# larskuenkel/iterative_cleaner

Hardware: AMD Instinct MI355X
Metric: profiles cleaned/sec (whole node) (higher is better)
Workload: dtype f64; 1 GPU; C2 360x3200x1024 (nsub x nchan x nbin), max_iter 5, thresholds 5/5, exact leastsq fit; fit_mode=exact, dedisp=shift, loops=3, fit_rounds=33, fit_tail_sweeps=694, parallelism=single

## Files before the change

iterative_cleaner_amd/csrc/ic_internal.h:

```cpp
#pragma once
#include <hip/hip_ext.h>
#include <hip/hip_runtime.h>
#include <stdint.h>

namespace icgpu {

struct PendingTiming {
    hipEvent_t a = nullptr, b = nullptr;
    int used = 0, extra = 0;
};
extern thread_local PendingTiming g_timing;
#define IC_GGL(K, GRID, BLOCK, SHM, ST, ...)                                                                 \
    do {                                                                                                    \
        if (::icgpu::g_timing.a && !::icgpu::g_timing.used) {                                               \
            ::icgpu::g_timing.used = 1;                                                                     \
            hipExtLaunchKernelGGL(K, GRID, BLOCK, SHM, ST, ::icgpu::g_timing.a, ::icgpu::g_timing.b, 0,      \
                                  __VA_ARGS__);                                                             \
        } else {                                                                                            \
            if (::icgpu::g_timing.a) ++::icgpu::g_timing.extra;                                             \
            hipLaunchKernelGGL(K, GRID, BLOCK, SHM, ST, __VA_ARGS__);                                       \
        }                                                                                                   \
    } while (0)

constexpr int kSuperBlock = 256;
// ... 160 lines not shown
    int32_t *info;
    const float *w0;
    const int32_t *shift;
    const double2 *tw, *tw_p2;
    const PwPlan *plan;
    int nsub, nchan, nbin;
    int pr_on;
    double pr_factor;
    int pr_start, pr_end;
    double *std_o, *mean_o, *fft_o, *ptp_o;
    int data_f64;
    int dtiled;
    const int32_t *list = nullptr;
    const unsigned long long *nctr = nullptr;
    const uint8_t *skip = nullptr;
    int chain = 1;
    int grid_cap = 0;
};
hipError_t launch_diag(hipStream_t st, const DiagArgs &a);
bool diag_list_supported(const DiagArgs &a);
size_t diag_lds_bytes(int nbin);
hipError_t launch_tnorm(hipStream_t st, const double *T64, const PwPlan *plan, int nleaf_ub, double *TT);
hipError_t launch_linestats(hipStream_t st, const LineStatsArgs &a, int which = 3);
hipError_t launch_combine(hipStream_t st, int nsub, int nchan, const uint8_t *valid, const int32_t *info,
                          const float *w0,
                          const double *std_d, const double *mean_d, const double *ptp_d, int ptp_f32,
                          const double *fft_d, const double *col_med, const double *col_mad,
                          const double *row_med, const double *row_mad, double chanthresh,
                          double subintthresh, double *test, float *W, float *hist, int iter,
                          int32_t *counters, int grid_cap = 0);
__host__ __device__ inline double2 ic_phasor0(int k, double d, int n)
{
    const double c = d * 8193.0;
    const double dh = c - (c - d);
    const double dl = d - dh;
    const double kk = (double)k, nn = (double)n;
    const double xh = kk * dh, xl = kk * dl;
    const double t = xh - nn * rint(xh * (1.0 / nn));
    const double y = (t + xl) * (4.0 / nn);
    const double q = rint(y);
    const double z = y - q;
    const double w = z * z;
    double sp = 0x1.aaec32af93359p-38;
    sp = -0x1.6fadb9f155744p-31 + w * sp;
    sp = 0x1.e8f434d018d63p-25 + w * sp;
    sp = -0x1.e3074fde8871fp-19 + w * sp;
    sp = 0x1.50783487ee782p-13 + w * sp;
    sp = -0x1.32d2cce62bd86p-8 + w * sp;
    sp = 0x1.466bc6775aae2p-4 + w * sp;
    sp = -0x1.4abbce625be53p-1 + w * sp;
    sp = 0x1.921fb54442d18p+0 + w * sp;
    const double sn = z * sp;
    double cp = 0x1.20c62c2f2d7f5p-34;
// ... 68 lines not shown
```

iterative_cleaner_amd/csrc/ic_kernels.hip:

```cpp
#include <algorithm>
#include <float.h>
#include <math.h>
#include <stdint.h>
#include <stdio.h>
#include <stdlib.h>

#include <type_traits>

#include "ic_internal.h"

namespace icgpu {

__device__ constexpr double kRdwarf = 3.834e-20;
__device__ constexpr double kRgiant = 1.304e19;

__device__ __forceinline__ void wave_sync()
{
    __builtin_amdgcn_fence(__ATOMIC_RELEASE, "wavefront");
    __builtin_amdgcn_wave_barrier();
    __builtin_amdgcn_fence(__ATOMIC_ACQUIRE, "wavefront");
}

constexpr int kDppXor1 = 0xB1, kDppXor2 = 0x4E, kDppHalfMirror = 0x141, kDppMirror = 0x140;

// ... 3928 lines not shown
        const double m = unkey64(wave_select(keys, n, idx, hist, lane));
        return f32 ? (double)(0.0f + (float)m) : 0.0 + m;
    }
    const unsigned long long klo = wave_select(keys, n, idx - 1, hist, lane);
    int le = 0;
    unsigned long long nxt = ~0ull;
    for (int j = lane; j < n; j += 64) {
        const unsigned long long k = keys[j];
        le += k <= klo;
        if (k > klo && k < nxt) nxt = k;
    }
    le = wave_sum_i(le);
    nxt = wave_min_u64(nxt);
    const unsigned long long khi = le > idx ? klo : nxt;
    const double lo = unkey64(klo), hi = unkey64(khi);
    if (f32) {
        const float t = (0.0f + (float)lo) + (float)hi;
        return (double)(t / 2.0f);
    }
    const double t = (0.0 + lo) + hi;
    return t / 2.0;
}

__global__ __launch_bounds__(256) void k_linestats(LineStatsArgs a, int rows, int len, int wpb, int per_wave)
{
    extern __shared__ __attribute__((aligned(16))) unsigned char lsm[];
    const int wave = threadIdx.x >> 6, lane = threadIdx.x & 63;
    const int line = blockIdx.x * wpb + wave;
    const int nl = 4 * (rows ? a.nsub : a.nchan);
    if (line >= nl || wave >= wpb) return;
    unsigned *hist = (unsigned *)(lsm + (size_t)wave * per_wave);
    unsigned long long *keys = (unsigned long long *)(lsm + (size_t)wave * per_wave + 1024);
    const int nline = rows ? a.nsub : a.nchan;
    const int diag = line / nline, idx = line % nline;
    const bool f32 = diag == 2 && a.ptp_f32, plain = diag == 3;
    int cnt = 0, nan = 0;
    for (int q0 = 0; q0 < len; q0 += 64) {
        const int q = q0 + lane;
        double d = 0.0;
        bool v = false;
        if (q < len) {
            const size_t kk = rows ? (size_t)idx * a.nchan + q : (size_t)q * a.nchan + idx;
            v = plain ? true : (a.valid[kk] != 0);
            d = diag == 0 ? a.std_d[kk] : diag == 1 ? a.mean_d[kk] : diag == 2 ? a.ptp_d[kk] : a.fft_d[kk];
        }
        const unsigned long long m = __ballot(v);
        if (v) keys[cnt + __popcll(m & ((1ull << lane) - 1ull))] = key64(d);
        nan |= v && isnan(d);
        cnt += __popcll(m);
    }
    nan = __any(nan);
// ... 1 lines not shown
    double med = NAN, mad = NAN;
    if (cnt > 0 && !nan) {
        med = wave_median(keys, cnt, f32, hist, lane);
        int rnan = 0;
        for (int j = lane; j < cnt; j += 64) {
            const double d = unkey64(keys[j]);
            const double r = f32 ? (double)fabsf((float)d - (float)med) : fabs(d - med);
            rnan |= isnan(r);
            keys[j] = key64(r);
        }
        rnan = __any(rnan);
        wave_sync();
        if (!rnan) mad = wave_median(keys, cnt, f32, hist, lane);
    }
    if (lane == 0) {
        if (!rows) {
            a.col_med[diag * a.nchan + idx] = med;
            a.col_mad[diag * a.nchan + idx] = mad;
        } else {
            a.row_med[diag * a.nsub + idx] = med;
            a.row_mad[diag * a.nsub + idx] = mad;
        }
    }
}


template <int W> struct GrpRed {
    unsigned long long *s;
    int wave, lane;
    __device__ unsigned long long min_u64(unsigned long long v)
    {
        v = wave_min_u64(v);
        if (lane == 0) s[wave] = v;
        __syncthreads();
        unsigned long long r = s[0];
#pragma unroll
        for (int i = 1; i < W; ++i) r = s[i] < r ? s[i] : r;
        __syncthreads();
        return r;
    }
    __device__ unsigned long long max_u64(unsigned long long v)
    {
        v = wave_max_u64(v);
        if (lane == 0) s[wave] = v;
        __syncthreads();
        unsigned long long r = s[0];
// ... 105 lines not shown
        const double m = unkey64(grp_select<W>(g, keys, n, idx, hist));
        return f32 ? (double)(0.0f + (float)m) : 0.0 + m;
    }
    const unsigned long long klo = grp_select<W>(g, keys, n, idx - 1, hist);
    int le = 0;
    unsigned long long nxt = ~0ull;
    for (int j = g.lane; j < n; j += 64) {
        const unsigned long long k = keys[j];
        le += k <= klo;
        if (k > klo && k < nxt) nxt = k;
    }
    le = g.sum_i(le);
    nxt = g.min_u64(nxt);
    const unsigned long long khi = le > idx ? klo : nxt;
    const double lo = unkey64(klo), hi = unkey64(khi);
    if (f32) {
        const float t = (0.0f + (float)lo) + (float)hi;
        return (double)(t / 2.0f);
    }
    const double t = (0.0 + lo) + hi;
    return t / 2.0;
}

template <int W> __global__ __launch_bounds__(64 * W) void k_linestats_grp(LineStatsArgs a, int rows, int len)
{
    extern __shared__ __attribute__((aligned(16))) unsigned char lsm[];
    const int wave = threadIdx.x >> 6, lane = threadIdx.x & 63;
    unsigned *hist = (unsigned *)lsm;
    GrpRed<W> g{(unsigned long long *)(lsm + 1024), wave, lane};
    const int nline = rows ? a.nsub : a.nchan;
    const int line = blockIdx.x;
    const int diag = line / nline, idx = line % nline;
    const bool f32 = diag == 2 && a.ptp_f32, plain = diag == 3;
    const int seg = (((len + W - 1) / W) + 63) & ~63;
    const int q0w = wave * seg, q1w = min(len, q0w + seg);
    unsigned long long *keys = (unsigned long long *)(lsm + 1024 + 16 * W) + q0w;
    int cnt = 0, nan = 0;
    for (int q0 = q0w; q0 < q1w; q0 += 64) {
        const int q = q0 + lane;
        double d = 0.0;
        bool v = false;
        if (q < q1w) {
            const size_t kk = rows ? (size_t)idx * a.nchan + q : (size_t)q * a.nchan + idx;
            v = plain ? true : (a.valid[kk] != 0);
            d = diag == 0 ? a.std_d[kk] : diag == 1 ? a.mean_d[kk] : diag == 2 ? a.ptp_d[kk] : a.fft_d[kk];
        }
        const unsigned long long m = __ballot(v);
        if (v) keys[cnt + __popcll(m & ((1ull << lane) - 1ull))] = key64(d);
        nan |= v && isnan(d);
        cnt += __popcll(m);
    }
    nan = g.sum_uniform(__any(nan) ? 1 : 0);
    const int ntot = g.sum_uniform(cnt);
    double med = NAN, mad = NAN;
    if (ntot > 0 && !nan) {
        med = grp_median<W>(g, keys, cnt, ntot, f32, hist);
        int rnan = 0;
        for (int j = lane; j < cnt; j += 64) {
            const double d = unkey64(keys[j]);
            const double r = f32 ? (double)fabsf((float)d - (float)med) : fabs(d - med);
            rnan |= isnan(r);
            keys[j] = key64(r);
        }
        rnan = g.sum_uniform(__any(rnan) ? 1 : 0);
        if (!rnan) mad = grp_median<W>(g, keys, cnt, ntot, f32, hist);
    }
    if (threadIdx.x == 0) {
        if (!rows) {
            a.col_med[diag * a.nchan + idx] = med;
            a.col_mad[diag * a.nchan + idx] = mad;
        } else {
            a.row_med[diag * a.nsub + idx] = med;
            a.row_mad[diag * a.nsub + idx] = mad;
        }
    }
}


__device__ __forceinline__ double scale_masked_d(double dv, bool valid, double med, double mad, double thr)
{
    if (!valid) return 0.0 + fabs(dv);
    const double r = dv - med;
    const double q = r / mad;
    const bool dom = !isfinite(q) || (fabs(r) * DBL_MIN >= fabs(mad));
    if (dom) return 0.0 + fabs(0.0 + r);
    const double aq = fabs(q);
    const double res = aq / thr;
    if (!isfinite(res) || aq * DBL_MIN >= fabs(thr)) return 0.0 + aq;
    return res;
}

__device__ __forceinline__ double scale_masked_f(float dv, bool valid, float med, float mad, double thr)
{
    if (!valid) return 0.0 + (double)fabsf(dv);
    const float r = dv - med;
    const float q = r / mad;
    const bool dom = !isfinite(q) || ((double)fabsf(r) * DBL_MIN >= (double)fabsf(mad));
    if (dom) return 0.0 + (double)fabsf(0.0f + r);
    const float aq = fabsf(q);
    const double res = (double)aq / thr;
// ... 4 lines not shown
__device__ __forceinline__ double scale_plain(double dv, double med, double mad, double thr)
{
    const double r = dv - med;
    const double q = r / mad;
    return fabs(q) / thr;
}

__device__ __forceinline__ double nanmax2(double a, double b)
{
    if (isnan(a) || isnan(b)) return NAN;
    return a > b ? a : b;
}

constexpr double kNearTie = 1e-9;


__global__ __launch_bounds__(256) void k_combine(
    int nsub, int nchan, const uint8_t *__restrict__ valid, const int32_t *__restrict__ info,
    const float *__restrict__ w0,
    const double *__restrict__ std_d, const double *__restrict__ mean_d, const double *__restrict__ ptp_d, int ptp_f32,
    const double *__restrict__ fft_d, const double *__restrict__ col_med, const double *__restrict__ col_mad,
    const double *__restrict__ row_med, const double *__restrict__ row_mad, double cth, double sth,
    double *__restrict__ test, float *__restrict__ W, float *__restrict__ hist, int iter,
    int32_t *__restrict__ counters)
{
    __shared__ int red[4][4];
    __shared__ unsigned long long dred[4];
    const size_t P = (size_t)nsub * nchan;
    int changed = 0, zero = 0, bad = 0, near = 0;
    unsigned long long diff = 0ull;
    const int hmax = iter < 64 ? iter : 64;
    for (size_t k = (size_t)blockIdx.x * blockDim.x + threadIdx.x; k < P; k += (size_t)gridDim.x * blockDim.x) {
        const int s = (int)(k / nchan), c = (int)(k % nchan);
        const bool v = valid[k] != 0;
        double S[4];
        S[0] = nanmax2(scale_masked_d(std_d[k], v, col_med[c], col_mad[c], cth),
                       scale_masked_d(std_d[k], v, row_med[s], row_mad[s], sth));
        S[1] = nanmax2(scale_masked_d(mean_d[k], v, col_med[nchan + c], col_mad[nchan + c], cth),
                       scale_masked_d(mean_d[k], v, row_med[nsub + s], row_mad[nsub + s], sth));
        S[2] = ptp_f32 ? nanmax2(scale_masked_f((float)ptp_d[k], v, (float)col_med[2 * nchan + c],
                                                (float)col_mad[2 * nchan + c], cth),
                                 scale_masked_f((float)ptp_d[k], v, (float)row_med[2 * nsub + s],
                                                (float)row_mad[2 * nsub + s], sth))
                       : nanmax2(scale_masked_d(ptp_d[k], v, col_med[2 * nchan + c], col_mad[2 * nchan + c], cth),
                                 scale_masked_d(ptp_d[k], v, row_med[2 * nsub + s], row_mad[2 * nsub + s], sth));
        S[3] = nanmax2(scale_plain(fft_d[k], col_med[3 * nchan + c], col_mad[3 * nchan + c], cth),
                       scale_plain(fft_d[k], row_med[3 * nsub + s], row_mad[3 * nsub + s], sth));
        double t;
        if (isnan(S[0]) || isnan(S[1]) || isnan(S[2]) || isnan(S[3])) {
            t = NAN;
// ... 11 lines not shown
        near += fabs(t - 1.0) <= kNearTie;
        const float wn = (t >= 1.0) ? 0.0f : w0[k];
        W[k] = wn;
        hist[(size_t)iter * P + k] = wn;
        changed += !(wn == hist[(size_t)(iter - 1) * P + k]);
        zero += (wn == 0.0f);
        if (info) {
            const int st = info[k];
            bad += (st < 1 || st > 4);
        }
        for (int h = 0; h < hmax; ++h)
            if (!(wn == hist[(size_t)h * P + k])) diff |= 1ull << h;
        for (int h = 64; h < iter; ++h)
            if (!(wn == hist[(size_t)h * P + k])) atomicOr(&counters[4 + h], 1);
    }
    for (int off = 32; off > 0; off >>= 1) {
        changed += __shfl_xor(changed, off);
        zero += __shfl_xor(zero, off);
        bad += __shfl_xor(bad, off);
        near += __shfl_xor(near, off);
        diff |= __shfl_xor(diff, off);
    }
    const int wave = threadIdx.x >> 6, nw = blockDim.x >> 6;
    if ((threadIdx.x & 63) == 0) {
        red[0][wave] = changed;
        red[1][wave] = zero;
        red[2][wave] = bad;
        red[3][wave] = near;
        dred[wave] = diff;
    }
    __syncthreads();
    if (threadIdx.x == 0) {
        int ch = 0, ze = 0, bd = 0, nt = 0;
        unsigned long long df = 0ull;
        for (int w = 0; w < nw; ++w) {
            ch += red[0][w];
            ze += red[1][w];
            bd += red[2][w];
            nt += red[3][w];
            df |= dred[w];
        }
        if (ch || ze)
            atomicAdd((unsigned long long *)counters, ((unsigned long long)(unsigned)ze << 32) | (unsigned)ch);
        if (bd) atomicAdd(&counters[2], bd);
        if (nt) atomicAdd(&counters[3], nt);
        for (int h = 0; h < hmax; ++h)
            if ((df >> h) & 1ull) atomicOr(&counters[4 + h], 1);
    }
}


__device__ __forceinline__ int geom_row_owner(const ShardGeom &g, int s)
{
    int r = 0;
    while (r + 1 < g.world && s >= g.row0[r + 1]) ++r;
    return r;
}
__device__ __forceinline__ int geom_chan_owner(const ShardGeom &g, int c)
{
    int r = 0;
    while (r + 1 < g.world && c >= g.chan0[r + 1]) ++r;
    return r;
}

__global__ __launch_bounds__(256) void k_pack_rows(ShardGeom g, int nchan_loc, const double *__restrict__ std_d,
                                                   const double *__restrict__ mean_d, const double *__restrict__ fft_d,
                                                   const double *__restrict__ ptp_d, const uint8_t *__restrict__ valid,
                                                   unsigned char *__restrict__ send)
{
    const size_t P = (size_t)g.nsub * nchan_loc;
    const size_t esz = valid ? 1 : 32;
// ... 476 lines not shown
    while (wpb > 1 && fixed + wpb * lay.per_wave > 150 * 1024) --wpb;
    const size_t shm = fixed + wpb * lay.per_wave;
    if (shm > 160 * 1024) return hipErrorInvalidValue;
    const unsigned grid = cap_grid(std::min<size_t>((P + wpb - 1) / wpb, 8192), a.grid_cap);
    IC_GGL(k_diag, dim3(grid), dim3(64 * wpb), shm, st, a);
    return hipGetLastError();
}

size_t diag_lds_bytes(int nbin)
{
    if (p2_supported(nbin)) return 0;
    const int nleaf_ub = nbin <= 128 ? 1 : (nbin / 64 + 1);
    const DiagLayout lay = diag_layout(nbin, nleaf_ub, nleaf_ub);
    return (size_t)lay.ntw * 16 + lay.per_wave;
}

hipError_t launch_tnorm(hipStream_t st, const double *T64, const PwPlan *plan, int nleaf_ub, double *TT)
{
    const size_t shm = (size_t)(nleaf_ub * 9 + nleaf_ub + 8) * 8;
    IC_GGL(k_tnorm, dim3(1), dim3(64), shm, st, T64, plan, TT);
    return hipGetLastError();
}

hipError_t launch_linestats(hipStream_t st, const LineStatsArgs &a, int which)
{
    for (int rows = 0; rows < 2; ++rows) {
        if (!((which >> rows) & 1)) continue;
        const int len = rows ? a.nchan : a.nsub;
        const int lines = 4 * (rows ? a.nsub : a.nchan);
        if (lines == 0 || len == 0) continue;
        if (lines < 8192 && len >= a.grp_minlen) {
            const int W = a.grp_waves;
            if (W == 4 || W == 8) {
                const int seg = (((len + W - 1) / W) + 63) & ~63;
                const size_t gshm = 1024 + 16 * (size_t)W + (size_t)W * seg * 8;
                if (gshm <= 160 * 1024) {
                    if (W == 4)
                        IC_GGL(k_linestats_grp<4>, dim3(lines), dim3(256), gshm, st, a, rows, len);
                    else
                        IC_GGL(k_linestats_grp<8>, dim3(lines), dim3(512), gshm, st, a, rows, len);
                    const hipError_t e = hipGetLastError();
                    if (e != hipSuccess) return e;
                    continue;
                }
            }
        }
        const int per_wave = 1024 + ((len * 8 + 15) / 16) * 16;
        int wpb = 4;
        while (wpb > 1 && (size_t)wpb * per_wave > 64 * 1024) --wpb;
        const size_t shm = (size_t)wpb * per_wave;
        if (shm > 160 * 1024) return hipErrorInvalidValue;
        IC_GGL(k_linestats, dim3(cdiv(lines, wpb)), dim3(64 * wpb), shm, st, a, rows, len, wpb,
                           per_wave);
        const hipError_t e = hipGetLastError();
        if (e != hipSuccess) return e;
    }
    return hipSuccess;
}

hipError_t launch_combine(hipStream_t st, int nsub, int nchan, const uint8_t *valid, const int32_t *info,
                          const float *w0,
                          const double *std_d, const double *mean_d, const double *ptp_d, int ptp_f32,
                          const double *fft_d, const double *col_med, const double *col_mad,
                          const double *row_med, const double *row_mad, double chanthresh,
                          double subintthresh, double *test, float *W, float *hist, int iter,
                          int32_t *counters, int grid_cap)
{
    const size_t P = (size_t)nsub * nchan;
    const unsigned grid = cap_grid(std::min<size_t>(cdiv(P, 256), 1024), grid_cap);
    IC_GGL(k_combine, dim3(grid), dim3(256), 0, st, nsub, nchan, valid, info, w0, std_d,
                       mean_d, ptp_d, ptp_f32, fft_d, col_med, col_mad, row_med, row_mad, chanthresh, subintthresh,
                       test, W, hist, iter, counters);
    return hipGetLastError();
}

hipError_t launch_residual(hipStream_t st, const float *D, const float *raw, const float *base, const double *T64,
                           const double *amp, const int32_t *info, const int32_t *shift, int nsub, int nchan,
                           int nbin, int ldD, int dtiled, int pr_on, double pr_factor, int pr_start, int pr_end,
                           float *R, int grid_cap)
{
    const size_t P = (size_t)nsub * nchan;
    if (!D && (!raw || !base)) return hipErrorInvalidValue;
    const unsigned grid = cap_grid(std::min<size_t>(cdiv(P, 4), 16384), grid_cap);
    IC_GGL(k_residual, dim3(grid), dim3(256), 0, st, D, raw, base, T64, amp, info, shift, P, nchan, nbin,
                       ldD, dtiled, pr_on, pr_factor, pr_start, pr_end, R);
    return hipGetLastError();
}

bool rotate_supported(int nbin) { return p2_supported(nbin); }

bool rotate_stats_supported(int nbin, bool data_f64) { return nbin == 1024 && !data_f64; }

__global__ __launch_bounds__(256) void k_rotate_identity(RotateArgs a)
{
    const int wave = threadIdx.x >> 6, lane = threadIdx.x & 63;
// ... 61 lines not shown
```

iterative_cleaner_amd/csrc/ic_session.hip:

```cpp
#include <hip/hip_runtime.h>
#include <math.h>
#include <stdarg.h>
#include <stdlib.h>
#include <stdio.h>
#include <sched.h>
#include <string.h>

#include <chrono>
#include <string>
#include <vector>

#include "../../include/iterative_cleaner.h"
#include "ic_comm.h"
#include "ic_internal.h"

using namespace icgpu;

namespace icgpu {
thread_local PendingTiming g_timing;
}

namespace {

thread_local std::string g_err;
// ... 11 lines not shown

int failed_session()
{
    return fail(IC_ESTATE, "session failed: a host wait timed out with its kernels possibly still running; destroy it");
}

#define CK(call)                                                                                  \
    do {                                                                                          \
        hipError_t e_ = (call);                                                                   \
        if (e_ != hipSuccess)                                                                     \
            return fail(IC_EHIP, "%s failed: %s (%s:%d)", #call, hipGetErrorString(e_), __FILE__, \
                        __LINE__);                                                                \
    } while (0)

const char *kKernelNames[K_COUNT] = {"k_chan_partials", "k_window",    "k_base",
                                     "k_fscrunch",      "k_tscrunch",  "k_fit_pass", "k_fit_state",
                                     "k_diag",          "k_linestats", "k_combine",  "k_residual",
                                     "k_fit_tail",      "k_sb_tree",   "k_shard_pack", "exchange",
                                     "k_tnorm",         "k_rotate"};

constexpr long kTailProfiles = 8192;
constexpr long kTailProfilesLarge = 4096;
constexpr long kTailProfilesLong = 12288;

struct Timed {
    int kid;
    hipEvent_t a, b;
};

struct Session {
    ic_params p{};
    int device = 0;
    hipStream_t stream = nullptr;
    size_t P = 0, N = 0, Ppad = 0;
    int ldD = 0;
    int nsb = 0, width = 0;
    bool uploaded = false, ran = false;
    int last_iter = 0;
    int rank = 0, world = 1;
    Comm *comm = nullptr;
    int nchan = 0;
    int c0 = 0;
    ShardGeom geom{};
    SbPlan plan_sb{};
    SbPlan plan_top{};
    int rows_own = 0, rows_pad = 0;
// ... 17 lines not shown
    int16_t *slot_q[2] = {nullptr, nullptr};
    float *slot_so[2] = {nullptr, nullptr};
    int slot_qsum[2] = {0, 0};
    int16_t *res_q = nullptr;
    float *res_so = nullptr;
    hipStream_t copy_stream = nullptr;
    int cur = 0, fifo[2] = {0, 0}, fifo_n = 0;
    bool ever_uploaded = false;
    float *F = nullptr, *wf = nullptr, *T = nullptr, *hist = nullptr;
    double *ptp = nullptr;
    uint8_t *valid = nullptr;
    int32_t *shift = nullptr, *win = nullptr, *wflag = nullptr, *info = nullptr, *counters = nullptr;
    double *part = nullptr, *part2 = nullptr, *wpart = nullptr, *T64 = nullptr, *amp = nullptr, *std_ = nullptr,
           *mean = nullptr, *fft = nullptr, *test = nullptr, *lstat = nullptr, *TT = nullptr,
           *T2 = nullptr;
    double2 *tw = nullptr, *tw_p2 = nullptr;
    PwPlan *plan = nullptr;
    FitStateArrays fs{};
    int32_t *lists = nullptr;
    int32_t *rcount = nullptr;
    int32_t *h_rcount = nullptr;
    int32_t *h_small = nullptr;
    int32_t *d_h_rcount = nullptr;
    void *fs_block = nullptr;
    int fit_rounds = 0;
    int plan_ub = 0;
    LineStatsArgs ls_knobs;
    long tail_threshold = kTailProfiles;
    bool diag_chain = true;
    int grid_cap = 0;
    double sync_timeout_s = 600.0;
    bool failed = false;
    bool comm_lost = false;
    int diag_fork = 3;
    int pr_lo = 0, pr_hi = 0;
    bool incr = true;
    uint8_t *exA = nullptr, *exF = nullptr;
    hipStream_t dstream = nullptr;
    hipEvent_t fork_ev = nullptr, join_ev = nullptr;
    uint8_t *late = nullptr;
    int fork_round = -1;
    bool tail_split = false;
    bool rot_stats = true;
    int tail_split_mode = IC_TAIL_SPLIT_AUTO;
    const int32_t *tail_list = nullptr;
    const unsigned long long *tail_cin = nullptr;
// ... 112 lines not shown
    using clk = std::chrono::steady_clock;
    const auto t0 = clk::now();
    const auto spin = kBusyPoll;
    const auto limit = std::chrono::duration<double>(s->sync_timeout_s);
    unsigned n = 0;
    while (__atomic_load_n(cnt, __ATOMIC_ACQUIRE) < 0) {
        const auto dt = clk::now() - t0;
        if (dt > limit) {
            s->failed = true;
            return hipErrorLaunchTimeOut;
        }
        if (dt > spin) {
            sched_yield();
            if (s->comm && (++n & 255) == 0 && s->comm->remote_error()) {
                s->failed = true;
                s->comm_lost = true;
                return hipErrorLaunchTimeOut;
            }
        }
    }
    return hipSuccess;
}

static hipError_t spin_sync(Session *s)
{
    hipError_t e = hipEventRecord(s->sev, s->stream);
    if (e != hipSuccess) return e;
    return poll_event(s, s->sev);
}

#define LAUNCH(S, KID, CALL) LAUNCH_ON(S, KID, (S)->stream, CALL)
#define LAUNCH_ON(S, KID, ST, CALL)                                            \
    do {                                                                       \
        Timed t_{KID, nullptr, nullptr};                                       \
        const bool tm_ = (S)->timing && ((S)->timing_only < 0 || (S)->timing_only == (KID)); \
        if (tm_) {                                                             \
            CK(take_event((S), &t_.a));                                        \
            CK(take_event((S), &t_.b));                                        \
            g_timing = PendingTiming{t_.a, t_.b, 0, 0};                        \
        }                                                                      \
        const hipError_t lc_ = (CALL);                                         \
        const PendingTiming pt_ = g_timing;                                    \
        g_timing = PendingTiming{};                                            \
        CK(lc_);                                                               \
        if (tm_ && pt_.used) {                                                 \
            if (pt_.extra) CK(hipEventRecord(t_.b, (ST)));                     \
// ... 57 lines not shown
    if (s->join_ev) (void)hipEventDestroy(s->join_ev);
    if (s->fork2_ev) (void)hipEventDestroy(s->fork2_ev);
    void *bufs[] = {s->late, s->exA, s->exF, s->D,     s->W,   s->base, s->base0, s->F,   s->wf,
                    s->T,    s->ptp,   s->hist, s->valid, s->win, s->info, s->comm ? nullptr : s->counters,
                    s->part, s->wpart, s->T64,  s->amp, s->std_, s->mean, s->fft,  s->test,
                    s->lstat, s->tw,   s->plan, s->fs_block, s->lists, s->rcount, s->tw_p2, s->part2,
                    s->wflag, s->TT, s->dr, s->Tc, s->R, s->zbase, s->zshift, s->ph, s->T2, s->fs.U, s->tmark,
                    s->dly, s->res_q, s->res_so};
    for (void *b : bufs)
        if (b) (void)hipFree(b);
    void *rbufs[] = {s->std_r, s->mean_r, s->fft_r, s->ptp_r, s->valid_r};
    for (void *b : rbufs)
        if (b) (void)hipFree(b);
    if (s->comm) {
        void *xbufs[] = {s->xw_send, s->xw_recv, s->xf_send, s->xf_recv, s->xwg_send, s->xwg_recv, s->xfg_send,
                         s->xfg_recv, s->xd_send, s->xd_recv, s->xr_send, s->xr_recv, s->counters};
        for (void *b : xbufs)
            if (b) s->comm->release(b);
        s->counters = nullptr;
        delete s->comm;
        s->comm = nullptr;
    }
    if (s->h_rcount) (void)hipHostFree(s->h_rcount);
    if (s->h_small) (void)hipHostFree(s->h_small);
    if (s->sev) (void)hipEventDestroy(s->sev);
    for (auto &e : s->epool) (void)hipEventDestroy(e);
    s->epool.clear();
    s->events.clear();
    if (s->stream) (void)hipStreamDestroy(s->stream);
}

__global__ void k_valid(const float *w0, uint8_t *valid, float *W, float *hist0, size_t P)
{
    const size_t k = (size_t)blockIdx.x * blockDim.x + threadIdx.x;
    if (k < P) {
        const float w = w0[k];
        valid[k] = (w != 0.0f);
        W[k] = w;
        hist0[k] = w;
    }
}

#define CM(S, call, what)                                                                         \
    do {                                                                                          \
        Timed t_{K_EXCHANGE, nullptr, nullptr};                                                   \
        const bool tm_ = (S)->timing && ((S)->timing_only < 0 || (S)->timing_only == K_EXCHANGE); \
// ... 274 lines not shown
    LineStatsArgs lr;
    lr.nsub = s->rows_own;
    lr.nchan = s->geom.nchan_g;
    lr.valid = s->valid_r;
    lr.std_d = s->std_r;
    lr.mean_d = s->mean_r;
    lr.fft_d = s->fft_r;
    lr.ptp_d = s->ptp_r;
    lr.ptp_f32 = la.ptp_f32;
    lr.grp_waves = la.grp_waves;
    lr.grp_minlen = la.grp_minlen;
    lr.col_med = lr.col_mad = nullptr;
    lr.row_med = s->xr_send;
    lr.row_mad = s->xr_send + 4 * s->rows_own;
    LAUNCH(s, K_LINESTATS, launch_linestats(s->stream, lr, 2));
    CM(s, s->comm->allgather(s->xr_send, s->xr_recv, sizeof(double) * 8 * s->rows_pad, s->stream), "row statistics");
    LAUNCH(s, K_SHARD_PACK, launch_unpack_rowstats(s->stream, s->geom, s->rows_pad, s->xr_recv, la.row_med, la.row_mad));
    return 0;
}

int fork_diag(Session *s, const DiagArgs &da, int r);
unsigned long long *tail_counter(Session *s) { return (unsigned long long *)(s->rcount + kRoundWords + 2); }

int run_fit(Session *s, const DiagArgs *fork)
{
    s->fork_round = -1;
    s->tail_split = false;
    const long P = (long)s->P;
    const int nbin = s->p.nbin;
    CK(launch_fit_init(s->stream, s->fs, P, s->rcount, kRoundWords + 2, fork ? s->late : nullptr));
    CK(launch_fit_prep(s->stream, s->fs, s->T64, nbin));
    unsigned long long *ctr = (unsigned long long *)s->rcount;
    unsigned *done = (unsigned *)(s->rcount + 2 * kMaxRounds);
    unsigned long long *tail_sweeps = tail_counter(s);
    int32_t *bufs[3] = {s->lists, s->lists + P, s->lists + 2 * P};
    const int32_t *cur = nullptr;
    const unsigned long long *cin = nullptr;
    long bound = P;
    int rounds = 0;
    bool tail = false;
    int flagged = -1;
    for (int r = 0;; ++r) {
        if (r >= kMaxRounds) return fail(IC_EHIP, "lmdif did not terminate after %d rounds", r);
        if (bound <= s->tail_threshold) {
            if (flagged >= 0) {
                if (int rc = fork_diag(s, *fork, flagged)) return rc;
                flagged = -1;
            }
            const bool split = fork && (s->tail_split_mode == IC_TAIL_SPLIT_ON ||
                                        (s->tail_split_mode == IC_TAIL_SPLIT_AUTO && nbin >= 2048));
            if (split && s->fork_round >= 0 && cur && !s->fftded) {
                CK(launch_mark_list(s->stream, cur, cin, P, bound, s->tmark, 1));
                CK(hipEventRecord(s->fork2_ev, s->stream));
// ... 287 lines not shown
        s->wg_blk = (s->rows_pad + 1) & ~1;
        s->fg_blk = ((long)s->rows_pad * (nbin + 1) + 1) & ~1L;
        struct {
            void **ptr;
            size_t bytes;
            const char *name;
        } xb[] = {{(void **)&s->xw_send, sizeof(double) * nsub * nbin, "window roots"},
                  {(void **)&s->xw_recv, sizeof(double) * world * s->rows_own * nbin, "owned window roots"},
                  {(void **)&s->xf_send, sizeof(double) * nsub * (nbin + 1), "fscrunch roots"},
                  {(void **)&s->xf_recv, sizeof(double) * world * s->rows_own * (nbin + 1), "owned fscrunch roots"},
                  {(void **)&s->xwg_send, sizeof(int32_t) * s->wg_blk, "owned windows"},
                  {(void **)&s->xwg_recv, sizeof(int32_t) * s->wg_blk * world, "gathered windows"},
                  {(void **)&s->xfg_send, sizeof(float) * s->fg_blk, "owned fscrunch rows"},
                  {(void **)&s->xfg_recv, sizeof(float) * s->fg_blk * world, "gathered fscrunch rows"},
                  {(void **)&s->xd_send, dsend, "diagnostics send"},
                  {(void **)&s->xd_recv, drecv, "diagnostics receive"},
                  {(void **)&s->xr_send, sizeof(double) * 8 * s->rows_pad, "row statistics"},
                  {(void **)&s->xr_recv, sizeof(double) * 8 * s->rows_pad * world, "gathered row statistics"},
                  {(void **)&s->counters, sizeof(int32_t) * (p.max_iter + 5), "counters"}};
        for (auto &b : xb)
            if (s->comm->alloc(b.ptr, b.bytes + 16) != 0 || !*b.ptr)
                return bail(fail(IC_ENOMEM, "exchange buffer (%s, %zu bytes) failed", b.name, b.bytes));
    } else {
        AL(s->counters, (size_t)(p.max_iter + 5));
    }
#undef AL
    if (hipHostMalloc((void **)&s->h_rcount, sizeof(int32_t) * kMaxRounds,
                      hipHostMallocMapped | hipHostMallocCoherent) != hipSuccess ||
        hipHostGetDevicePointer((void **)&s->d_h_rcount, s->h_rcount, 0) != hipSuccess)
        return bail(fail(IC_ENOMEM, "hipHostMalloc(round counts) failed"));
    if (hipEventCreateWithFlags(&s->sev, hipEventDisableTiming) != hipSuccess)
        return bail(fail(IC_EHIP, "hipEventCreate failed"));
    if (hipHostMalloc((void **)&s->h_small, sizeof(int32_t) * ((size_t)p.max_iter + 20)) != hipSuccess)
        return bail(fail(IC_ENOMEM, "hipHostMalloc(readback) failed"));
    if (exact) {
        const size_t dstride = ((P * 8 + 255) / 256) * 256, istride = ((P * 4 + 255) / 256) * 256;
        if (hipMalloc(&s->fs_block, 21 * dstride + 5 * istride) != hipSuccess)
            return bail(fail(IC_ENOMEM, "hipMalloc(fit state) failed"));
        char *b = (char *)s->fs_block;
        double **dp[] = {&s->fs.x,     &s->fs.fnorm, &s->fs.par,   &s->fs.delta,   &s->fs.diag, &s->fs.xnorm,
                         &s->fs.acnorm, &s->fs.J0,   &s->fs.f0,    &s->fs.aj,      &s->fs.r,    &s->fs.Jn0,
                         &s->fs.qtf,   &s->fs.gnorm, &s->fs.x2,    &s->fs.pnorm,   &s->fs.wa1,  &s->fs.xa,
                         &s->fs.o_fnorm, &s->fs.o_acnorm, &s->fs.o_sum};
        for (auto *q : dp) { *q = (double *)b; b += dstride; }
        int32_t **ip[] = {&s->fs.iter, &s->fs.nfev, &s->fs.mode, &s->fs.slow, (int32_t **)&s->fs.p0};
        for (auto *q : ip) { *q = (int32_t *)b; b += istride; }
        s->fs.T64 = s->T64;
// ... 459 lines not shown
            std::swap(s->ph, s->slot_ph[slot]);
            s->delay2 = nullptr;
        } else if (s->slot_dmode[slot] == 2) {
            std::swap(s->dly, s->slot_dly[slot]);
            s->delay2 = s->dly;
        }
        if (s->slot_dmode[slot]) s->delays_set = true;
        s->slot_dmode[slot] = 0;
    }
    if (!s->uploaded) return fail(IC_ESTATE, "ic_run before ic_upload");
    if (s->events.size() > 4096)
        if (int rc = collect_timing(s)) return rc;
    if (s->fftded && !s->delays_set) return fail(IC_ESTATE, "ic_run before ic_set_delays (dedisp_mode FFT)");
    if (s->fftded && !rot_stats_on(s) && !s->R && dalloc(&s->R, s->N) != hipSuccess) {
        s->R = nullptr;
        return fail(IC_ENOMEM, "hipMalloc(R: %zu floats) failed", s->N);
    }
    if (s->tmark) CK(hipMemsetAsync(s->tmark, 0, s->P, s->stream));
    const ic_params &p = s->p;
    const int nsub = p.nsub, nchan = s->nchan, nbin = p.nbin;
    int pr_start = p.pr_start < 0 ? 0 : (p.pr_start > nbin ? nbin : p.pr_start);
    int pr_end = p.pr_end < 0 ? 0 : (p.pr_end > nbin ? nbin : p.pr_end);
    s->stats = ic_run_stats{};
    if (int rc = prepare(s)) return rc;
    LineStatsArgs la;
    la.nsub = nsub;
    la.nchan = nchan;
    la.valid = s->valid;
    la.std_d = s->std_;
    la.mean_d = s->mean;
    la.fft_d = s->fft;
    la.ptp_d = s->ptp;
    la.ptp_f32 = !p.data_f64;
    la.grp_waves = s->ls_knobs.grp_waves;
    la.grp_minlen = s->ls_knobs.grp_minlen;
    la.col_med = s->lstat;
    la.col_mad = s->lstat + 4 * nchan;
    la.row_med = s->lstat + 8 * nchan;
    la.row_mad = s->lstat + 8 * nchan + 4 * nsub;
    int32_t *cnt = s->h_small;
    s->bad_fits.clear();
    int x = 0, loops = -1, n_iter = 0, converged = 0;
    CK(hipMemsetAsync(tail_counter(s), 0, sizeof(unsigned long long), s->stream));
    while (x < p.max_iter) {
        x += 1;
        ++n_iter;
        if (int rc = iteration_template(s, n_iter)) return rc;
        DiagArgs da = diag_args(s, pr_start, pr_end);
        DiagArgs ds = da;
        if (s->fftded) {
            ds.mode = DIAG_STATS;
            ds.D = s->R;
            ds.ldD = nbin;
            ds.dtiled = 0;
        }
        s->pr_lo = pr_start;
        s->pr_hi = pr_end;
        if (p.fit_mode == IC_FIT_EXACT) {
            const bool fork = s->diag_fork > 0 && s->dstream && s->late && diag_list_supported(ds);
            if (int rc = run_fit(s, fork ? &ds : nullptr)) return rc;
        } else {
            LAUNCH(s, K_TNORM, launch_tnorm(s->stream, s->T64, s->plan, s->plan_ub, s->TT));
        }
// ... 18 lines not shown
            da = ds;
        }
        if (rot_stats_on(s)) {
            if (s->fork_round >= 0) CK(hipStreamWaitEvent(s->stream, s->join_ev, 0));
        } else if (s->tail_split) {
            DiagArgs b = da;
            b.list = s->tail_list;
            b.nctr = s->tail_cin;
            LAUNCH(s, K_DIAG, launch_diag(s->stream, b));
            CK(hipStreamWaitEvent(s->stream, s->join_ev, 0));
            CK(launch_mark_list(s->stream, s->tail_list, s->tail_cin, (long)s->P, s->tail_bound, s->tmark, 0));
        } else if (s->fork_round >= 0) {
            DiagArgs b = da;
            b.list = s->lists + 2 * s->P;
            b.nctr = (const unsigned long long *)s->rcount + s->fork_round;
            LAUNCH(s, K_DIAG, launch_diag(s->stream, b));
            CK(hipStreamWaitEvent(s->stream, s->join_ev, 0));
        } else {
            LAUNCH(s, K_DIAG, launch_diag(s->stream, da));
        }
        LAUNCH(s, K_LINESTATS, launch_linestats(s->stream, la, s->comm ? 1 : 3));
        if (s->comm)
            if (int rc = shard_rowstats(s, la)) return rc;
        CK(hipMemsetAsync(s->counters, 0, sizeof(int32_t) * (p.max_iter + 5), s->stream));
        LAUNCH(s, K_COMBINE,
               launch_combine(s->stream, nsub, nchan, s->valid, s->info, s->w0, s->std_, s->mean, s->ptp, la.ptp_f32,
                              s->fft,
                              la.col_med, la.col_mad, la.row_med, la.row_mad, p.chanthresh, p.subintthresh,
                              s->test, s->W, s->hist, n_iter, s->counters, s->grid_cap));
        if (s->comm)
            CM(s, s->comm->allreduce_sum_i32(s->counters, (size_t)(n_iter + 4), s->stream), "convergence counters");
        CK(hipMemcpyAsync(cnt, s->counters, sizeof(int32_t) * (n_iter + 4), hipMemcpyDeviceToHost,
                          s->stream));
        CK(spin_sync(s));
        if (changed_out) changed_out[n_iter - 1] = cnt[0];
        if (nzero_out) nzero_out[n_iter - 1] = cnt[1];
        s->bad_fits.push_back(cnt[2]);
        s->stats.near_threshold = cnt[3];
        for (int h = 0; h < n_iter; ++h)
            if (cnt[4 + h] == 0) {
                loops = x;
                converged = 1;
                x = 1000000;
            }
    }
    if (x == p.max_iter) loops = p.max_iter;
    s->last_iter = n_iter;
    if (test_out && n_iter > 0)
        CK(hipMemcpyAsync(test_out, s->test, sizeof(double) * s->P, hipMemcpyDeviceToHost, s->stream));
    if (weights_out)
        CK(hipMemcpyAsync(weights_out, s->W, sizeof(float) * s->P, hipMemcpyDeviceToHost, s->stream));
    {
        int32_t *moves = s->h_small + p.max_iter + 6;
        unsigned long long *tsw = (unsigned long long *)(s->h_small + ((p.max_iter + 9) & ~1));
        CK(hipMemcpyAsync(moves, s->wflag + nsub, sizeof *moves, hipMemcpyDeviceToHost, s->stream));
        CK(hipMemcpyAsync(tsw, tail_counter(s), sizeof *tsw, hipMemcpyDeviceToHost, s->stream));
        CK(spin_sync(s));
        s->stats.window_moves = *moves;
        s->stats.fit_tail_sweeps += (int64_t)tsw[0];
    }
    if (loops_out) *loops_out = loops;
    if (n_iter_out) *n_iter_out = n_iter;
    s->stats.iterations = n_iter;
    if (converged_out) *converged_out = converged;
    s->ran = n_iter > 0;
    return IC_OK;
}

}

extern "C" {

int ic_run(void *session, double *test_out, float *weights_out, int32_t *loops_out, int32_t *changed_out,
           int32_t *nzero_out, int32_t *n_iter_out, int32_t *converged_out)
{
// ... 559 lines not shown
    Session *s = (Session *)h;
    struct Guard {
        Session *s;
        ~Guard() { ic_session_destroy(s); }
    } guard{s};
    s->dtiled = 0;
    const size_t P = s->P, row = sizeof(float) * (size_t)nbin;
    std::vector<double> t64(s->ldD, 0.0);
    for (int i = 0; i < nbin; ++i) t64[i] = (double)T[i];
    CK(hipMemcpyAsync(s->T64, t64.data(), sizeof(double) * s->ldD, hipMemcpyHostToDevice, s->stream));
    CK(hipMemcpyAsync(s->T2, t64.data(), sizeof(double) * nbin, hipMemcpyHostToDevice, s->stream));
    CK(hipMemcpyAsync(s->T2 + nbin, t64.data(), sizeof(double) * nbin, hipMemcpyHostToDevice, s->stream));
    CK(hipMemsetAsync(s->shift, 0, sizeof(int32_t) * s->nchan, s->stream));
    CK(hipMemsetAsync(s->base0, 0, sizeof(float) * P, s->stream));
    {
        std::vector<float> ones(P, 1.0f);
        CK(hipMemcpyAsync(s->w0, ones.data(), sizeof(float) * P, hipMemcpyHostToDevice, s->stream));
        CK(hipStreamSynchronize(s->stream));
    }
    CK(hipMemsetAsync(s->raw, 0, sizeof(float) * s->N, s->stream));
    CK(hipMemcpyAsync(s->raw, profiles, row * nprof, hipMemcpyHostToDevice, s->stream));
    if (fit_mode == IC_FIT_EXACT) {
        CK(hipMemcpy2DAsync(s->D, sizeof(float) * s->ldD, s->raw, row, row, P, hipMemcpyDeviceToDevice, s->stream));
        if (int r = run_fit(s, nullptr)) return r;
    } else {
        CK(launch_tnorm(s->stream, s->T64, s->plan, s->plan_ub, s->TT));
        DiagArgs da = diag_args(s, 0, 0);
        CK(launch_diag(s->stream, da));
    }
    if (amp_out) CK(hipMemcpyAsync(amp_out, s->amp, sizeof(double) * nprof, hipMemcpyDeviceToHost, s->stream));
    if (info_out) CK(hipMemcpyAsync(info_out, s->info, sizeof(int32_t) * nprof, hipMemcpyDeviceToHost, s->stream));
    if (resid_out) {
        float *R = nullptr;
        CK(hipMalloc((void **)&R, sizeof(float) * s->N));
        hipError_t e = launch_residual(s->stream, s->D, s->raw, s->base0, s->T64, s->amp, s->info, s->shift, p.nsub,
                                       s->nchan, nbin, s->ldD, s->dtiled, 0, 1.0, 0, 0, R, s->grid_cap);
        if (e == hipSuccess) e = hipMemcpyAsync(resid_out, R, row * nprof, hipMemcpyDeviceToHost, s->stream);
        if (e == hipSuccess) e = hipStreamSynchronize(s->stream);
        (void)hipFree(R);
        if (e != hipSuccess) return fail(IC_EHIP, "ic_fit_profiles residual: %s", hipGetErrorString(e));
    }
    CK(hipStreamSynchronize(s->stream));
    return IC_OK;
}

}
// ... 1 lines not shown
```

Measured before the change: 45.38 million profiles/s.

## Fuse row/column linestats launches and hand off convergence counters via mapped host memory

Row and column line statistics are now computed by one combined kernel launch instead of two. The combine kernel's last-finishing block, chosen by an atomic ticket, writes the convergence counters, window moves and tail-sweep count straight into coherent mapped host memory with a tag, then zeroes the counters. The host polls that tag instead of issuing a memset, a memcpy and an event sync for each iteration. The next fit-init is queued before polling so the GPU has work while the host waits. This cuts per-iteration launch and round-trip overhead, at the cost of system-scope memory ordering that must be correct, host busy-polling, and a changed fit_init placement.

```diff
diff --git a/iterative_cleaner_amd/csrc/ic_internal.h b/iterative_cleaner_amd/csrc/ic_internal.h
--- a/iterative_cleaner_amd/csrc/ic_internal.h
+++ b/iterative_cleaner_amd/csrc/ic_internal.h
@@ -206,13 +206,22 @@
 size_t diag_lds_bytes(int nbin);
 hipError_t launch_tnorm(hipStream_t st, const double *T64, const PwPlan *plan, int nleaf_ub, double *TT);
 hipError_t launch_linestats(hipStream_t st, const LineStatsArgs &a, int which = 3);
+constexpr int kHandTag = 0, kHandMoves = 1, kHandSweeps = 2 , kHandCounters = 4;
+struct CombineHandoff {
+    int32_t *host = nullptr;
+    unsigned *ticket = nullptr;
+    const int32_t *moves = nullptr;
+    const unsigned long long *sweeps = nullptr;
+    unsigned tag = 0;
+    int nread = 0, nzero = 0;
+};
 hipError_t launch_combine(hipStream_t st, int nsub, int nchan, const uint8_t *valid, const int32_t *info,
                           const float *w0,
                           const double *std_d, const double *mean_d, const double *ptp_d, int ptp_f32,
                           const double *fft_d, const double *col_med, const double *col_mad,
                           const double *row_med, const double *row_mad, double chanthresh,
                           double subintthresh, double *test, float *W, float *hist, int iter,
-                          int32_t *counters, int grid_cap = 0);
+                          int32_t *counters, int grid_cap = 0, const CombineHandoff &ho = CombineHandoff{});
 __host__ __device__ inline double2 ic_phasor0(int k, double d, int n)
 {
     const double c = d * 8193.0;
diff --git a/iterative_cleaner_amd/csrc/ic_kernels.hip b/iterative_cleaner_amd/csrc/ic_kernels.hip
--- a/iterative_cleaner_amd/csrc/ic_kernels.hip
+++ b/iterative_cleaner_amd/csrc/ic_kernels.hip
@@ -3974,11 +3974,11 @@
     return t / 2.0;
 }
 
-__global__ __launch_bounds__(256) void k_linestats(LineStatsArgs a, int rows, int len, int wpb, int per_wave)
-{
-    extern __shared__ __attribute__((aligned(16))) unsigned char lsm[];
+__device__ __forceinline__ void linestats_wave(const LineStatsArgs &a, int rows, int len, int wpb, int per_wave,
+                                               int blk, unsigned char *lsm)
+{
     const int wave = threadIdx.x >> 6, lane = threadIdx.x & 63;
-    const int line = blockIdx.x * wpb + wave;
+    const int line = blk * wpb + wave;
     const int nl = 4 * (rows ? a.nsub : a.nchan);
     if (line >= nl || wave >= wpb) return;
     unsigned *hist = (unsigned *)(lsm + (size_t)wave * per_wave);
@@ -4026,6 +4026,12 @@
             a.row_mad[diag * a.nsub + idx] = mad;
         }
     }
+}
+
+__global__ __launch_bounds__(256) void k_linestats(LineStatsArgs a, int rows, int len, int wpb, int per_wave)
+{
+    extern __shared__ __attribute__((aligned(16))) unsigned char lsm[];
+    linestats_wave(a, rows, len, wpb, per_wave, blockIdx.x, lsm);
 }
 
 
@@ -4177,14 +4183,13 @@
     return t / 2.0;
 }
 
-template <int W> __global__ __launch_bounds__(64 * W) void k_linestats_grp(LineStatsArgs a, int rows, int len)
-{
-    extern __shared__ __attribute__((aligned(16))) unsigned char lsm[];
+template <int W>
+__device__ __forceinline__ void linestats_grp(const LineStatsArgs &a, int rows, int len, int line, unsigned char *lsm)
+{
     const int wave = threadIdx.x >> 6, lane = threadIdx.x & 63;
     unsigned *hist = (unsigned *)lsm;
     GrpRed<W> g{(unsigned long long *)(lsm + 1024), wave, lane};
     const int nline = rows ? a.nsub : a.nchan;
-    const int line = blockIdx.x;
     const int diag = line / nline, idx = line % nline;
     const bool f32 = diag == 2 && a.ptp_f32, plain = diag == 3;
     const int seg = (((len + W - 1) / W) + 63) & ~63;
@@ -4231,6 +4236,31 @@
     }
 }
 
+template <int W> __global__ __launch_bounds__(64 * W) void k_linestats_grp(LineStatsArgs a, int rows, int len)
+{
+    extern __shared__ __attribute__((aligned(16))) unsigned char lsm[];
+    linestats_grp<W>(a, rows, len, blockIdx.x, lsm);
+}
+
+struct LineKind {
+    int rows, len, grouped, nblk, wpb, per_wave;
+};
+template <int W>
+__global__ __launch_bounds__(W ? 64 * W : 256) void k_linestats_both(LineStatsArgs a, LineKind k0, LineKind k1)
+{
+    extern __shared__ __attribute__((aligned(16))) unsigned char lsm[];
+    const bool first = (int)blockIdx.x < k0.nblk;
+    const int blk = first ? (int)blockIdx.x : (int)blockIdx.x - k0.nblk;
+    const int rows = first ? k0.rows : k1.rows, len = first ? k0.len : k1.len;
+    if constexpr (W > 0) {
+        if (first ? k0.grouped : k1.grouped) {
+            linestats_grp<W>(a, rows, len, blk, lsm);
+            return;
+        }
+    }
+    linestats_wave(a, rows, len, first ? k0.wpb : k1.wpb, first ? k0.per_wave : k1.per_wave, blk, lsm);
+}
+
 
 __device__ __forceinline__ double scale_masked_d(double dv, bool valid, double med, double mad, double thr)
 {
@@ -4281,10 +4311,11 @@
     const double *__restrict__ fft_d, const double *__restrict__ col_med, const double *__restrict__ col_mad,
     const double *__restrict__ row_med, const double *__restrict__ row_mad, double cth, double sth,
     double *__restrict__ test, float *__restrict__ W, float *__restrict__ hist, int iter,
-    int32_t *__restrict__ counters)
+    int32_t *__restrict__ counters, CombineHandoff ho)
 {
     __shared__ int red[4][4];
     __shared__ unsigned long long dred[4];
+    __shared__ bool last_blk;
     const size_t P = (size_t)nsub * nchan;
     int changed = 0, zero = 0, bad = 0, near = 0;
     unsigned long long diff = 0ull;
@@ -4342,6 +4373,7 @@
         diff |= __shfl_xor(diff, off);
     }
     const int wave = threadIdx.x >> 6, nw = blockDim.x >> 6;
+    if (ho.host && iter > 64) asm volatile("s_waitcnt vmcnt(0)" ::: "memory");
     if ((threadIdx.x & 63) == 0) {
         red[0][wave] = changed;
         red[1][wave] = zero;
@@ -4366,7 +4398,33 @@
         if (nt) atomicAdd(&counters[3], nt);
         for (int h = 0; h < hmax; ++h)
             if ((df >> h) & 1ull) atomicOr(&counters[4 + h], 1);
-    }
+        if (ho.host) {
+            asm volatile("s_waitcnt vmcnt(0)" ::: "memory");
+            const unsigned t = __hip_atomic_fetch_add(ho.ticket, 1u, __ATOMIC_RELAXED, __HIP_MEMORY_SCOPE_AGENT);
+            last_blk = t == gridDim.x - 1;
+        }
+    }
+    if (!ho.host) return;
+    __syncthreads();
+    if (!last_blk) return;
+    __builtin_amdgcn_fence(__ATOMIC_ACQUIRE, "agent");
+    for (int q = threadIdx.x; q < ho.nzero; q += blockDim.x) {
+        if (q < ho.nread)
+            __hip_atomic_store(ho.host + kHandCounters + q,
+                               __hip_atomic_load(counters + q, __ATOMIC_RELAXED, __HIP_MEMORY_SCOPE_AGENT),
+                               __ATOMIC_RELAXED, __HIP_MEMORY_SCOPE_SYSTEM);
+        __hip_atomic_store(counters + q, 0, __ATOMIC_RELAXED, __HIP_MEMORY_SCOPE_AGENT);
+    }
+    if (threadIdx.x == 0) {
+        __hip_atomic_store(ho.host + kHandMoves, *ho.moves, __ATOMIC_RELAXED, __HIP_MEMORY_SCOPE_SYSTEM);
+        __hip_atomic_store((unsigned long long *)(ho.host + kHandSweeps), *ho.sweeps, __ATOMIC_RELAXED,
+                           __HIP_MEMORY_SCOPE_SYSTEM);
+        __hip_atomic_store(ho.ticket, 0u, __ATOMIC_RELAXED, __HIP_MEMORY_SCOPE_AGENT);
+    }
+    asm volatile("s_waitcnt vmcnt(0)" ::: "memory");
+    __syncthreads();
+    if (threadIdx.x == 0)
+        __hip_atomic_store((unsigned *)(ho.host + kHandTag), ho.tag, __ATOMIC_RELAXED, __HIP_MEMORY_SCOPE_SYSTEM);
 }
 
 
@@ -4889,36 +4947,75 @@
     return hipGetLastError();
 }
 
+struct LinePlan {
+    int rows, len, lines, W, wpb, per_wave;
+    size_t shm;
+};
+static LinePlan plan_lines(const LineStatsArgs &a, int rows)
+{
+    LinePlan p{};
+    p.rows = rows;
+    p.len = rows ? a.nchan : a.nsub;
+    p.lines = 4 * (rows ? a.nsub : a.nchan);
+    const int W = a.grp_waves;
+    if (p.lines < 8192 && p.len >= a.grp_minlen && (W == 4 || W == 8)) {
+        const int seg = (((p.len + W - 1) / W) + 63) & ~63;
+        const size_t gshm = 1024 + 16 * (size_t)W + (size_t)W * seg * 8;
+        if (gshm <= 160 * 1024) {
+            p.W = W;
+            p.shm = gshm;
+        }
+    }
+    p.per_wave = 1024 + ((p.len * 8 + 15) / 16) * 16;
+    return p;
+}
+static void plan_waves(LinePlan &p, int wpb_max)
+{
+    if (p.W) return;
+    p.wpb = wpb_max;
+    while (p.wpb > 1 && (size_t)p.wpb * p.per_wave > 64 * 1024) --p.wpb;
+    p.shm = (size_t)p.wpb * p.per_wave;
+}
+
+static hipError_t launch_linestats_both(hipStream_t st, const LineStatsArgs &a)
+{
+    LinePlan p[2] = {plan_lines(a, 1), plan_lines(a, 0)};
+    if (p[1].len > p[0].len) std::swap(p[0], p[1]);
+    const int W = std::max(p[0].W, p[1].W);
+    LineKind k[2];
+    for (int q = 0; q < 2; ++q) {
+        plan_waves(p[q], W ? W : 4);
+        if (p[q].shm > 160 * 1024) return hipErrorInvalidValue;
+        k[q] = LineKind{p[q].rows, p[q].len, p[q].W != 0, p[q].W ? p[q].lines : (int)cdiv(p[q].lines, p[q].wpb),
+                        p[q].wpb, p[q].per_wave};
+    }
+    const size_t shm = std::max(p[0].shm, p[1].shm);
+    const dim3 grid((unsigned)(k[0].nblk + k[1].nblk));
+    if (W == 8)
+        IC_GGL(k_linestats_both<8>, grid, dim3(512), shm, st, a, k[0], k[1]);
+    else if (W == 4)
+        IC_GGL(k_linestats_both<4>, grid, dim3(256), shm, st, a, k[0], k[1]);
+    else
+        IC_GGL(k_linestats_both<0>, grid, dim3(256), shm, st, a, k[0], k[1]);
+    return hipGetLastError();
+}
+
 hipError_t launch_linestats(hipStream_t st, const LineStatsArgs &a, int which)
 {
+    if (which == 3 && a.nsub > 0 && a.nchan > 0) return launch_linestats_both(st, a);
     for (int rows = 0; rows < 2; ++rows) {
         if (!((which >> rows) & 1)) continue;
-        const int len = rows ? a.nchan : a.nsub;
-        const int lines = 4 * (rows ? a.nsub : a.nchan);
-        if (lines == 0 || len == 0) continue;
-        if (lines < 8192 && len >= a.grp_minlen) {
-            const int W = a.grp_waves;
-            if (W == 4 || W == 8) {
-                const int seg = (((len + W - 1) / W) + 63) & ~63;
-                const size_t gshm = 1024 + 16 * (size_t)W + (size_t)W * seg * 8;
-                if (gshm <= 160 * 1024) {
-                    if (W == 4)
-                        IC_GGL(k_linestats_grp<4>, dim3(lines), dim3(256), gshm, st, a, rows, len);
-                    else
-                        IC_GGL(k_linestats_grp<8>, dim3(lines), dim3(512), gshm, st, a, rows, len);
-                    const hipError_t e = hipGetLastError();
-                    if (e != hipSuccess) return e;
-                    continue;
-                }
-            }
-        }
-        const int per_wave = 1024 + ((len * 8 + 15) / 16) * 16;
-        int wpb = 4;
-        while (wpb > 1 && (size_t)wpb * per_wave > 64 * 1024) --wpb;
-        const size_t shm = (size_t)wpb * per_wave;
-        if (shm > 160 * 1024) return hipErrorInvalidValue;
-        IC_GGL(k_linestats, dim3(cdiv(lines, wpb)), dim3(64 * wpb), shm, st, a, rows, len, wpb,
-                           per_wave);
+        LinePlan p = plan_lines(a, rows);
+        if (p.lines == 0 || p.len == 0) continue;
+        plan_waves(p, 4);
+        if (p.shm > 160 * 1024) return hipErrorInvalidValue;
+        if (p.W == 4)
+            IC_GGL(k_linestats_grp<4>, dim3(p.lines), dim3(256), p.shm, st, a, rows, p.len);
+        else if (p.W == 8)
+            IC_GGL(k_linestats_grp<8>, dim3(p.lines), dim3(512), p.shm, st, a, rows, p.len);
+        else
+            IC_GGL(k_linestats, dim3(cdiv(p.lines, p.wpb)), dim3(64 * p.wpb), p.shm, st, a, rows, p.len, p.wpb,
+                   p.per_wave);
         const hipError_t e = hipGetLastError();
         if (e != hipSuccess) return e;
     }
@@ -4931,13 +5028,15 @@
                           const double *fft_d, const double *col_med, const double *col_mad,
                           const double *row_med, const double *row_mad, double chanthresh,
                           double subintthresh, double *test, float *W, float *hist, int iter,
-                          int32_t *counters, int grid_cap)
-{
+                          int32_t *counters, int grid_cap, const CombineHandoff &ho)
+{
+    if (ho.host && (!ho.ticket || !ho.moves || !ho.sweeps || ho.tag == 0 || ho.nread > ho.nzero))
+        return hipErrorInvalidValue;
     const size_t P = (size_t)nsub * nchan;
     const unsigned grid = cap_grid(std::min<size_t>(cdiv(P, 256), 1024), grid_cap);
     IC_GGL(k_combine, dim3(grid), dim3(256), 0, st, nsub, nchan, valid, info, w0, std_d,
                        mean_d, ptp_d, ptp_f32, fft_d, col_med, col_mad, row_med, row_mad, chanthresh, subintthresh,
-                       test, W, hist, iter, counters);
+                       test, W, hist, iter, counters, ho);
     return hipGetLastError();
 }
 
diff --git a/iterative_cleaner_amd/csrc/ic_session.hip b/iterative_cleaner_amd/csrc/ic_session.hip
--- a/iterative_cleaner_amd/csrc/ic_session.hip
+++ b/iterative_cleaner_amd/csrc/ic_session.hip
@@ -57,6 +57,8 @@
 constexpr long kTailProfiles = 8192;
 constexpr long kTailProfilesLarge = 4096;
 constexpr long kTailProfilesLong = 12288;
+
+static size_t hand_words(int max_iter) { return ((size_t)max_iter + 5 + 1 + 3) & ~(size_t)3; }
 
 struct Timed {
     int kid;
@@ -120,6 +122,8 @@
     int32_t *h_rcount = nullptr;
     int32_t *h_small = nullptr;
     int32_t *d_h_rcount = nullptr;
+    int32_t *h_hand = nullptr, *d_h_hand = nullptr;
+    unsigned hand_tag = 0;
     void *fs_block = nullptr;
     int fit_rounds = 0;
     int plan_ub = 0;
@@ -278,6 +282,22 @@
     return hipSuccess;
 }
 
+static hipError_t poll_tag(Session *s, const int32_t *word, unsigned tag)
+{
+    using clk = std::chrono::steady_clock;
+    const auto t0 = clk::now();
+    const auto limit = std::chrono::duration<double>(s->sync_timeout_s);
+    while ((unsigned)__atomic_load_n(word, __ATOMIC_ACQUIRE) != tag) {
+        const auto dt = clk::now() - t0;
+        if (dt > limit) {
+            s->failed = true;
+            return hipErrorLaunchTimeOut;
+        }
+        if (dt > kBusyPoll) sched_yield();
+    }
+    return hipSuccess;
+}
+
 static hipError_t spin_sync(Session *s)
 {
     hipError_t e = hipEventRecord(s->sev, s->stream);
@@ -381,6 +401,7 @@
         s->comm = nullptr;
     }
     if (s->h_rcount) (void)hipHostFree(s->h_rcount);
+    if (s->h_hand) (void)hipHostFree(s->h_hand);
     if (s->h_small) (void)hipHostFree(s->h_small);
     if (s->sev) (void)hipEventDestroy(s->sev);
     for (auto &e : s->epool) (void)hipEventDestroy(e);
@@ -701,13 +722,19 @@
 int fork_diag(Session *s, const DiagArgs &da, int r);
 unsigned long long *tail_counter(Session *s) { return (unsigned long long *)(s->rcount + kRoundWords + 2); }
 
+int queue_fit_init(Session *s)
+{
+    if (s->p.fit_mode != IC_FIT_EXACT) return 0;
+    CK(launch_fit_init(s->stream, s->fs, (long)s->P, s->rcount, kRoundWords + 2, s->late));
+    return 0;
+}
+
 int run_fit(Session *s, const DiagArgs *fork)
 {
     s->fork_round = -1;
     s->tail_split = false;
     const long P = (long)s->P;
     const int nbin = s->p.nbin;
-    CK(launch_fit_init(s->stream, s->fs, P, s->rcount, kRoundWords + 2, fork ? s->late : nullptr));
     CK(launch_fit_prep(s->stream, s->fs, s->T64, nbin));
     unsigned long long *ctr = (unsigned long long *)s->rcount;
     unsigned *done = (unsigned *)(s->rcount + 2 * kMaxRounds);
@@ -1041,7 +1068,12 @@
             if (s->comm->alloc(b.ptr, b.bytes + 16) != 0 || !*b.ptr)
                 return bail(fail(IC_ENOMEM, "exchange buffer (%s, %zu bytes) failed", b.name, b.bytes));
     } else {
-        AL(s->counters, (size_t)(p.max_iter + 5));
+        AL(s->counters, hand_words(p.max_iter));
+        if (hipHostMalloc((void **)&s->h_hand, sizeof(int32_t) * (kHandCounters + (size_t)p.max_iter + 5),
+                          hipHostMallocMapped | hipHostMallocCoherent) != hipSuccess ||
+            hipHostGetDevicePointer((void **)&s->d_h_hand, s->h_hand, 0) != hipSuccess)
+            return bail(fail(IC_ENOMEM, "hipHostMalloc(counter hand-off) failed"));
+        memset(s->h_hand, 0, sizeof(int32_t) * (kHandCounters + (size_t)p.max_iter + 5));
     }
 #undef AL
     if (hipHostMalloc((void **)&s->h_rcount, sizeof(int32_t) * kMaxRounds,
@@ -1547,6 +1579,7 @@
     int pr_start = p.pr_start < 0 ? 0 : (p.pr_start > nbin ? nbin : p.pr_start);
     int pr_end = p.pr_end < 0 ? 0 : (p.pr_end > nbin ? nbin : p.pr_end);
     s->stats = ic_run_stats{};
+    if (int rc = queue_fit_init(s)) return rc;
     if (int rc = prepare(s)) return rc;
     LineStatsArgs la;
     la.nsub = nsub;
@@ -1563,7 +1596,17 @@
     la.col_mad = s->lstat + 4 * nchan;
     la.row_med = s->lstat + 8 * nchan;
     la.row_mad = s->lstat + 8 * nchan + 4 * nsub;
-    int32_t *cnt = s->h_small;
+    const bool hand = !s->comm;
+    const int32_t *cnt = hand ? s->h_hand + kHandCounters : s->h_small;
+    CombineHandoff ho;
+    if (hand) {
+        ho.host = s->d_h_hand;
+        ho.ticket = (unsigned *)(s->counters + p.max_iter + 5);
+        ho.moves = s->wflag + nsub;
+        ho.sweeps = tail_counter(s);
+        ho.nzero = p.max_iter + 5;
+        CK(hipMemsetAsync(s->counters, 0, sizeof(int32_t) * hand_words(p.max_iter), s->stream));
+    }
     s->bad_fits.clear();
     int x = 0, loops = -1, n_iter = 0, converged = 0;
     CK(hipMemsetAsync(tail_counter(s), 0, sizeof(unsigned long long), s->stream));
@@ -1628,17 +1671,28 @@
         LAUNCH(s, K_LINESTATS, launch_linestats(s->stream, la, s->comm ? 1 : 3));
         if (s->comm)
             if (int rc = shard_rowstats(s, la)) return rc;
-        CK(hipMemsetAsync(s->counters, 0, sizeof(int32_t) * (p.max_iter + 5), s->stream));
+        if (hand) {
+            if (++s->hand_tag == 0) ++s->hand_tag;
+            ho.tag = s->hand_tag;
+            ho.nread = n_iter + 4;
+        } else {
+            CK(hipMemsetAsync(s->counters, 0, sizeof(int32_t) * (p.max_iter + 5), s->stream));
+        }
         LAUNCH(s, K_COMBINE,
                launch_combine(s->stream, nsub, nchan, s->valid, s->info, s->w0, s->std_, s->mean, s->ptp, la.ptp_f32,
                               s->fft,
                               la.col_med, la.col_mad, la.row_med, la.row_mad, p.chanthresh, p.subintthresh,
-                              s->test, s->W, s->hist, n_iter, s->counters, s->grid_cap));
-        if (s->comm)
+                              s->test, s->W, s->hist, n_iter, s->counters, s->grid_cap, ho));
+        if (x < p.max_iter)
+            if (int rc = queue_fit_init(s)) return rc;
+        if (hand) {
+            CK(poll_tag(s, s->h_hand + kHandTag, ho.tag));
+        } else {
             CM(s, s->comm->allreduce_sum_i32(s->counters, (size_t)(n_iter + 4), s->stream), "convergence counters");
-        CK(hipMemcpyAsync(cnt, s->counters, sizeof(int32_t) * (n_iter + 4), hipMemcpyDeviceToHost,
-                          s->stream));
-        CK(spin_sync(s));
+            CK(hipMemcpyAsync(s->h_small, s->counters, sizeof(int32_t) * (n_iter + 4), hipMemcpyDeviceToHost,
+                              s->stream));
+            CK(spin_sync(s));
+        }
         if (changed_out) changed_out[n_iter - 1] = cnt[0];
         if (nzero_out) nzero_out[n_iter - 1] = cnt[1];
         s->bad_fits.push_back(cnt[2]);
@@ -1656,7 +1710,11 @@
         CK(hipMemcpyAsync(test_out, s->test, sizeof(double) * s->P, hipMemcpyDeviceToHost, s->stream));
     if (weights_out)
         CK(hipMemcpyAsync(weights_out, s->W, sizeof(float) * s->P, hipMemcpyDeviceToHost, s->stream));
-    {
+    if (hand && n_iter > 0) {
+        s->stats.window_moves = s->h_hand[kHandMoves];
+        s->stats.fit_tail_sweeps += (int64_t) * (const unsigned long long *)(s->h_hand + kHandSweeps);
+        if ((test_out && n_iter > 0) || weights_out) CK(spin_sync(s));
+    } else {
         int32_t *moves = s->h_small + p.max_iter + 6;
         unsigned long long *tsw = (unsigned long long *)(s->h_small + ((p.max_iter + 9) & ~1));
         CK(hipMemcpyAsync(moves, s->wflag + nsub, sizeof *moves, hipMemcpyDeviceToHost, s->stream));
@@ -2262,6 +2320,7 @@
     CK(hipMemcpyAsync(s->raw, profiles, row * nprof, hipMemcpyHostToDevice, s->stream));
     if (fit_mode == IC_FIT_EXACT) {
         CK(hipMemcpy2DAsync(s->D, sizeof(float) * s->ldD, s->raw, row, row, P, hipMemcpyDeviceToDevice, s->stream));
+        if (int r = queue_fit_init(s)) return r;
         if (int r = run_fit(s, nullptr)) return r;
     } else {
         CK(launch_tnorm(s->stream, s->T64, s->plan, s->plan_ub, s->TT));
```

Measured after the change: 45.74 million profiles/s, median of 6. No clear change (+0.8%).
